# yeeecheng/DA-CLIP

Hardware: AMD Instinct MI355X
Metric: restored images/sec @256x256, 100 IR-SDE steps; PSNR vs ref; 1/2/4/8 MI355X (higher is better)
Workload: dtype fp16; 1 GPU; deraining-shaped synthetic batch, 256x256, batch=8/GPU, 100 IR-SDE posterior steps, hipGraph loop (BASELINE configs[1]); model=universal-ir, batch_per_gpu=8, global_batch=8, resolution=256, sde_steps=100, sampler=posterior, parallelism=dp1

## Files before the change

da-clip_amd/csrc/kernels.h:

```cpp
#pragma once
#include <hip/hip_runtime.h>
#include <stdint.h>

namespace dac {

enum Act { ACT_NONE = 0, ACT_SILU = 1, ACT_GELU = 2, ACT_GEGLU = 3 };

struct ConvArgs {
  const void* x1; const void* x2;
  int ld1, ld2, C1, Cin;
  int Hs, Ws, up;
  int B, Ho, Wo, Cout, K;
  const void* w;
  const float* bias;
  const float* ss;
  int ss_ld;
  const void* res1; int ldr1;
  const void* res2; int ldr2;
  const float* bbias; int bb_ld;
  void* y; int ldy;
  int act;
  int amode;
  long long w_bstride;
  const void* zero;
  const float* ln_g;
  float ln_eps;
  int cwrap;
  const void* w2;
  const float* bias2;
  int w2_dual;
  void* y2; int ldy2;
  const float* lnf_cs;
  int lnf_n;
  float lnf_eps;
  const float* gna_stats;
  const float* gna_g;
  const float* gna_b;
  int gna_groups;
  int dbuf;
  int gna_nb;
  float gna_eps;
  uint8_t* ys8;
  const uint8_t* xs8;
  int uph;
  int ksplit;
  float* part;
  const void* w_gs;
  const float* b_gs;
  unsigned long long* stamp;
};
bool conv_lnf_ok(const ConvArgs& a, int elem_bytes);
bool conv_gna_ok(const ConvArgs& a, int elem_bytes);
template <typename T>
const float* groupnorm_stats(const void* x, int B, int HW, int C, int groups, float eps, float* part,
                             hipStream_t st);
template <typename T>
int layernorm_gnstats(const void* x, int ldx, void* y, int ldy, const float* g, const float* b, int rows, int C,
                      float eps, int HW, int groups, float* part, bool launch, hipStream_t st);
size_t layernorm_gnstats_ws_floats(int B, int HW, int groups);
bool conv_res_fusable(const ConvArgs& a);

inline bool conv3w_ok(const ConvArgs& a) {
  return a.Cin == 64 && a.Cout == 64 && a.K == 576 && a.cwrap == 0 && !a.y2 && (!a.ss || (a.ss_ld % 4 == 0 && ((uintptr_t)a.ss & 15) == 0)) && a.amode == 0 && a.w_bstride == 0 &&
         !a.ln_g && (a.act == ACT_NONE || a.act == ACT_SILU) && a.Wo >= 64 && a.Wo % 64 == 0 &&
         (a.C1 >= a.Cin || a.C1 % 32 == 0) && a.ldy % 8 == 0 && a.ld1 % 8 == 0 &&
         (a.C1 >= a.Cin || a.ld2 % 8 == 0) && (!a.res1 || a.ldr1 % 8 == 0) && !a.res2 && !a.bbias && !(a.ss && a.res1);
}
template <typename T>
void conv(const ConvArgs& a, int kh, int kw, int stride, int pad, hipStream_t st);
struct RbArgs {
  const void* x1; const void* x2;
  int ld1, ld2, C1, Cin;
  int B, H, W;
  const void* w1;
  const void* w2;
  const void* wr;
  const float* ss; int ss_ld;
  void* y; int ldy;
  unsigned long long* stamp;
};
bool rbfuse_pays(const RbArgs& a);
bool rbfuse_ok(const RbArgs& a);
template <typename T>
void rbfuse(const RbArgs& a, hipStream_t st);
bool conv3r_ok(const ConvArgs& a);
template <typename T>
void conv3r(const ConvArgs& a, hipStream_t st);
bool conv7_ok(const ConvArgs& a);
template <typename T>
void conv7(const ConvArgs& a, hipStream_t st);
bool conv3n_ok(const ConvArgs& a);
template <typename T>
void conv3n(const ConvArgs& a, hipStream_t st);
bool conv_down_ok(const ConvArgs& a);
template <typename T>
void conv_down(const ConvArgs& a, hipStream_t st);
int conv_variant(const ConvArgs& a, int kh, int elem_bytes);

bool conv8_ok(const ConvArgs& a, int kh, int kw, int s, int p);
template <typename T>
void conv8(const ConvArgs& a, int kh, int kw, int s, int p, const uint8_t* w8, const uint8_t* ws8, int Kp,
           hipStream_t st);
bool conv_q8out_ok(const ConvArgs& a);
int conv_split_k(const ConvArgs& a, int elem_bytes, long rows);
bool conv3_split_ok(const ConvArgs& a, int elem_bytes);
int conv3_split_k(const ConvArgs& a, int elem_bytes, int ks);
template <typename T>
void conv_part_reduce(const ConvArgs& a, hipStream_t st);
bool conv_uph_ok(const ConvArgs& a, int elem_bytes);
bool conv3q_ok(const ConvArgs& a);
template <typename T>
void conv3q(const ConvArgs& a, const uint8_t* q8w, const uint8_t* q8s, hipStream_t st);

template <typename T>
void layernorm(const void* x, int ldx, void* y, int ldy, const void* res, int ldr,
               const float* g, const float* b, int rows, int C, float eps, hipStream_t st);

template <typename T>
void groupnorm(const void* x, void* y, const float* g, const float* b, int B, int HW, int C,
               int groups, float eps, float* stats_ws, hipStream_t st);

template <typename T>
void flash_attn_d32(const void* qkv, void* o, int B, int L, int H, float scale, hipStream_t st);
template <typename T>
void flash_attn_d32_v(const void* qkv, void* o, int B, int L, int H, float scale, int variant, hipStream_t st);
extern int g_flash_old;

template <typename T>
void text_embed(const int64_t* tok, const float* emb, const float* pos, void* x, int N, int L, int D, int V,
                hipStream_t st);
template <typename T>
void eot_gather(const int64_t* tok, const void* x, void* out, int N, int L, int D, hipStream_t st);
void degradation_probs(const float* degra, const float* text, int B, int K, int E, float* probs,
                       int32_t* argmax, hipStream_t st);

template <typename T>
void small_mha(const void* qkv, void* o, int B, int L, int H, int D, int causal, hipStream_t st);

template <typename T>
void linear_attention_weff(const void* qkv, const float* wout, void* weff, int B, int HW, int C,
                           float* ws, hipStream_t st, float hw_scale = 0.f);
template <typename T>
void linear_attention_fused(const void* x, const void* wqkv, const float* wout, const float* bout,
                            const float* gout, void* weff, void* y, int B, int HW, int C, float* ws,
                            hipStream_t st, float qshift = 0.f);
size_t linear_attention_fused_ws_floats(int B, int HW);
size_t linear_attention_ws_floats(int B, int HW);

void small_linear(const float* x, int ldx, const float* W, const float* b, float* y, int ldy,
                  int R, int I, int O, int pre_act, int post_act, const float* add, int add_ld,
                  int add_mod, hipStream_t st);
void sinus_embedding(float* out, int R, int B, int nf, double t0, double dt, double scale,
                     hipStream_t st);
void round_bf16_rows(float* y, int ld, size_t rows, int C, hipStream_t st);
void ss_fill(float* ss, int C, float scale_m1, const float* shift, hipStream_t st);
void set_u64x2(uint64_t* p, uint64_t a, uint64_t b, hipStream_t st);
void stamp_init(unsigned long long* s, size_t n, hipStream_t st);
void softmax_mul(const float* x, const float* v, float* y, int R, int C, hipStream_t st);

template <typename T>
void unet_prep(const float* xt, const float* mu, void* x, int B, int H, int W, int Hp, int Wp,
               hipStream_t st);

template <typename T>
void unet_out(const void* y, int ld, float* eps, int B, int H, int W, int Hp, int Wp,
              hipStream_t st);

struct StepCoef { float sbar, ea, t1, t2, std, theta, sigma2, dt, sigma_sqrt_dt; };
template <typename T>
void sde_step(int mode, float* x, const float* mu, const void* eps, int ld, int Hp, int Wp,
              const float* z, const uint64_t* seedp, uint32_t tag, StepCoef c, int B, int H,
              int W, hipStream_t st, void* xin = nullptr);
bool sde_step_fuses(int ld, int H, int W, int Hp, int Wp);

void tile_gather(const float* src, float* dst, const int32_t* ys_dev, const int32_t* xs_dev,
                 const int32_t* xs_host, int ny, int nx, int H, int W, int th, int tw, int k0, int nk,
                 hipStream_t st);
void tile_blend(const float* tiles, float* out, const int32_t* ys_dev, const int32_t* xs_dev,
                const int32_t* xs_host, int B, int ny, int nx, int H, int W, int th, int tw, int ov,
                hipStream_t st);
void rows_gather(const float* src, float* dst, int rows, int ld, int k0, int per, hipStream_t st);

template <typename T>
void vit_prep(const float* img, void* x, int B, int S, hipStream_t st);
template <typename T>
void vit_patches(const float* img, void* x, int B, int S, int P, hipStream_t st);
template <typename T>
void vit_embed(const void* patch, const float* cls, const float* pos, void* tok, int B, int L,
               int D, hipStream_t st);
template <typename T>
void rows_to_f32(const void* x, int ld, float* y, int R, int D, hipStream_t st);

bool image_metrics_ok(int B, int C, int H, int W, int cb);
size_t image_metrics_ws_bytes(int B, int C, int H, int W, int cb);
void image_metrics(const float* out, const float* gt, int B, int C, int H, int W, int cb,
                   unsigned char* out_u8, unsigned char* gt_u8, double* results, void* ws,
                   hipStream_t st);

}
```

da-clip_amd/csrc/rbfuse.hip:

```cpp
#include "conv_impl.h"

namespace dac {

namespace {
constexpr unsigned RBF_OOB = 0x80000000u;
DEV int rbf_phys(int p) { return p ^ ((p >> 2) & 1); }
DEV int rbf_chunk(int P, int q) { return q ^ ((P >> 2) & 7); }
DEV int rbf_off(int p, int q) {
  const int P = rbf_phys(p);
  return P * 128 + (rbf_chunk(P, q) << 4);
}

template <int CIN> struct RBF {
  static constexpr int NSRC = CIN / 64;
  static constexpr int SW = CIN == 64 ? 128 : 64;
  static constexpr int NG = SW / 64;
  static constexpr int JT = NG;
  static constexpr int OPW = 16 * JT;
  static constexpr int NGW = 4 / NG;
  static constexpr int NC1 = CIN / 32;
  static constexpr int XPX = SW + 4, NIX = (XPX + 7) / 8, XHALF = NIX * 1024, XROW = NSRC * XHALF;
  static constexpr int HPX = SW + 2, NIH = (HPX + 7) / 8, HROW = NIH * 1024;
  static constexpr int XS = 5, HS = 4;
  static constexpr int OFF_H = XS * XROW, OFF_T = OFF_H + HS * HROW;
  static constexpr int SMEM = OFF_T + 512;
  static_assert(SMEM <= 160 * 1024, "LDS");
};

template <typename T> DEV void store4_g(T* p, const float* v) {
  typedef T T4 __attribute__((ext_vector_type(4)));
  T4 o;
#pragma unroll
  for (int e = 0; e < 4; ++e) o[e] = (T)v[e];
  *reinterpret_cast<T4*>(p) = o;
}
template <typename T> DEV void st_lds(char* p, const float* v, int n) {
  if (n == 8) {
    typedef T T8 __attribute__((ext_vector_type(8)));
    T8 o;
#pragma unroll
    for (int e = 0; e < 8; ++e) o[e] = (T)v[e];
    *reinterpret_cast<T8*>(p) = o;
  } else {
    typedef T T4 __attribute__((ext_vector_type(4)));
    T4 o;
#pragma unroll
    for (int e = 0; e < 4; ++e) o[e] = (T)v[e];
    *reinterpret_cast<T4*>(p) = o;
  }
}
}

static int g_rbfuse_on = getenv("DAC_RBFUSE") ? atoi(getenv("DAC_RBFUSE")) : 1;
extern "C" void dac_rbfuse_enable(int on) { g_rbfuse_on = on; }

bool rbfuse_pays(const RbArgs& a) {
  const size_t px = (size_t)a.B * a.H * a.W, img = (size_t)256 * 256;
  if (g_rbfuse_on == 3) return a.Cin == 64 || px <= 2 * img;
  return true;
}

bool rbfuse_ok(const RbArgs& a) {
  if (!g_rbfuse_on || !(a.Cin == 64 || a.Cin == 128)) return false;
  const int SW = a.Cin == 64 ? RBF<64>::SW : RBF<128>::SW;
  if ((a.Cin == 128) != (a.wr != nullptr)) return false;
  const bool one = a.x2 == nullptr || a.C1 >= a.Cin;
  if (!one && !(a.C1 == 64 && a.Cin == 128 && a.ld2 % 8 == 0)) return false;
  return a.W % SW == 0 && a.W >= 256 && a.ld1 % 8 == 0 && a.ldy % 8 == 0 && a.ss_ld % 4 == 0 &&
         ((size_t)a.H * a.W + 1) * a.ld1 * 2 < ((size_t)1 << 31) &&
         (one || ((size_t)a.H * a.W + 1) * a.ld2 * 2 < ((size_t)1 << 31));
}

template <typename T, int CIN>
__global__ void __launch_bounds__(512, 2) rbfuse_kernel(RbArgs a, int RB) {
  kernarg_touch<sizeof(RbArgs) + 4>();
  StampGuard stamp_guard(a.stamp);
  using G = RBF<CIN>;
  constexpr int JT = G::JT, SW = G::SW, NC1 = G::NC1, EV = 4 * JT;
  constexpr bool FUSE = CIN == 128;
  __shared__ __attribute__((aligned(1024))) char smem[G::SMEM];
  const int lane = threadIdx.x & 63;
  const int wave = __builtin_amdgcn_readfirstlane(threadIdx.x >> 6);
  const bool conv1 = wave < 4;
  const int wl = wave & 3;
  const int g = wl / G::NGW, ob = G::OPW * (wl % G::NGW);
  const int lr = lane & 15, lg = lane >> 4;
  const int nb = ob + EV * lg;

  const int nbands = gridDim.x;
  const int bid = nbands % 8 == 0 ? (blockIdx.x & 7) * (nbands >> 3) + (blockIdx.x >> 3) : blockIdx.x;
  const int S = a.W / SW, nrb = a.H / RB;
  const int strip = bid % S, rb = (bid / S) % nrb, img = bid / (S * nrb);
  const int x0 = strip * SW, r0 = rb * RB;
  const bool lpad = x0 == 0, rpad = x0 + SW == a.W;

  char* xring = smem;
  char* hring = smem + G::OFF_H;
  float* terms = reinterpret_cast<float*>(smem + G::OFF_T);
  if (threadIdx.x < 64) {
    const int n = threadIdx.x;
    float sc = 1.f + a.ss[(size_t)img * a.ss_ld + n], sh = a.ss[(size_t)img * a.ss_ld + 64 + n];
    epi_fold(0.f, sc, sh, true);
    terms[n] = sc;
    terms[64 + n] = sh;
  }

  const bool one = a.x2 == nullptr || a.C1 >= a.Cin;
  const int ldb0 = a.ld1 * 2, ldb1 = one ? ldb0 : a.ld2 * 2;
  const char* xsrc0 = reinterpret_cast<const char*>(a.x1) + (size_t)img * a.H * a.W * ldb0 - 2 * ldb0;
  const char* xsrc1 = one ? xsrc0 + 128
                          : reinterpret_cast<const char*>(a.x2) + (size_t)img * a.H * a.W * ldb1 - 2 * ldb1;
  const int xb0 = (a.H * a.W + 2) * ldb0, xb1 = (a.H * a.W + 2) * ldb1 - (one ? 128 : 0);
  auto xslot = [&](int row) { return xring + ((row + 10) % G::XS) * G::XROW; };
  auto issue_x = [&](int ir) {
    const bool ok = (unsigned)ir < (unsigned)a.H;
    char* dst = xslot(ir);
    int lane = threadIdx.x & 63;
    asm volatile("" : "+v"(lane));
    constexpr int NQ = G::NSRC * G::NIX;
#pragma unroll
    for (int k = 0; k < (NQ + 3) / 4; ++k) {
      const int q = wl + 4 * k;
      if (q < NQ) {
        const bool h1 = q >= G::NIX;
        const int qq = h1 ? q - G::NIX : q, ldb = h1 ? ldb1 : ldb0;
        const int P = 8 * qq + (lane >> 3), p = rbf_phys(P);
        const bool pad = p >= SW + 4 || (lpad && p < 2) || (rpad && p >= SW + 2);
        const int v = (ok && !pad) ? p * ldb + rbf_chunk(P, lane & 7) * 16 : (int)RBF_OOB;
        buf_lds16(h1 ? xsrc1 : xsrc0, h1 ? xb1 : xb0, dst + q * 1024, v, ok ? (ir * a.W + x0) * ldb : 0);
      }
    }
  };

  auto quad_base = [&](int u) {
    const int q = lr + u;
    return (64 * g + 4 * q) * 128 + ((q & 1) << 7) + ((lg ^ ((16 * g + q) & 7)) << 4);
  };
  const int bq0 = quad_base(0), bq1 = quad_base(1);
  auto foff = [&](int b0, int b1, int s, int c) {
    const int base = s < 4 ? b0 : b1;
    return base ^ ((s & 3) << 7) ^ (c << 6);
  };

  const int nsteps = RB + 3;
  if (conv1) {
    u32x4 W[9 * NC1][JT];
    {
      const T* w = reinterpret_cast<const T*>(a.w1);
#pragma unroll
      for (int j = 0; j < JT; ++j) {
        const int n = JT == 2 ? ob + 8 * (lr >> 2) + 4 * j + (lr & 3) : ob + lr;
#pragma unroll
        for (int ks = 0; ks < 9 * NC1; ++ks)
          W[ks][j] = *reinterpret_cast<const u32x4*>(w + (size_t)n * (9 * CIN) + (ks / NC1) * CIN + (ks % NC1) * 32 + 8 * lg);
      }
    }
    __builtin_amdgcn_s_waitcnt(0x0F70);
    issue_x(r0 - 2);
    issue_x(r0 - 1);
    issue_x(r0);
    int eoff[3], fo[2][6];
#pragma unroll
    for (int kw = 0; kw < 3; ++kw) eoff[kw] = rbf_off(lr < 8 ? SW + 1 + kw : kw, lg);
#pragma unroll
    for (int c = 0; c < 2; ++c)
#pragma unroll
      for (int s = 0; s < 6; ++s) fo[c][s] = foff(bq0, bq1, s + 1, c);
    for (int st = 0; st < nsteps; ++st) {
      const int t = r0 - 1 + st;
      asm volatile("s_waitcnt vmcnt(0) lgkmcnt(0)" ::: "memory");
      __builtin_amdgcn_s_barrier();
      asm volatile("" ::: "memory");
      if (t + 2 <= r0 + RB + 1) issue_x(t + 2);
      if (t > r0 + RB) continue;
      char* hdst = hring + (t & 3) * G::HROW;
      if ((unsigned)t >= (unsigned)a.H) {
        for (int i = threadIdx.x; i < G::HROW / 16; i += 256) reinterpret_cast<u32x4*>(hdst)[i] = u32x4{0u, 0u, 0u, 0u};
        continue;
      }
      f32x4 acc[4][JT], acce = f32x4{0.f, 0.f, 0.f, 0.f};
#pragma unroll
      for (int j = 0; j < JT; ++j)
#pragma unroll
        for (int i = 0; i < 4; ++i) acc[i][j] = f32x4{0.f, 0.f, 0.f, 0.f};
      if constexpr (CIN == 128) {
        constexpr int NGR = 3 * NC1;
        u32x4 F2[2][6];
        auto gsrc = [&](int gg) { return xslot(t + gg / NC1 - 1) + ((gg % NC1) >> 1) * G::XHALF; };
        auto ldF = [&](int gg, int h) __attribute__((always_inline)) {
          const char* hr = gsrc(gg);
          const int c = (gg % NC1) & 1;
#pragma unroll
          for (int s = 0; s < 6; ++s) F2[h][s] = *reinterpret_cast<const u32x4*>(hr + fo[c][s]);
        };
        ldF(0, 0);
#pragma unroll
        for (int gg = 0; gg < NGR; ++gg) {
          const int kh = gg / NC1, c32 = gg % NC1, c = c32 & 1;
          const char* hr = gsrc(gg);
          if (gg + 1 < NGR) ldF(gg + 1, (gg + 1) & 1);
          __builtin_amdgcn_sched_barrier(0);
#pragma unroll
          for (int kw = 0; kw < 3; ++kw)
#pragma unroll
            for (int i = 0; i < 4; ++i) Mma<T>::run(acc[i][0], W[(kh * 3 + kw) * NC1 + c32][0], F2[gg & 1][i + kw]);
#pragma unroll
          for (int kw = 0; kw < 3; ++kw) {
            const u32x4 E = *reinterpret_cast<const u32x4*>(hr + (eoff[kw] ^ (c << 6)));
            Mma<T>::run(acce, W[(kh * 3 + kw) * NC1 + c32][0], E);
          }
        }
      } else {
        constexpr int NGR = 3 * NC1;
        auto gsrc = [&](int gg) { return xslot(t + gg / NC1 - 1) + ((gg % NC1) >> 1) * G::XHALF; };
        u32x4 F[6];
        {
          const char* hr0 = gsrc(0);
#pragma unroll
          for (int s = 0; s < 6; ++s) F[s] = *reinterpret_cast<const u32x4*>(hr0 + fo[0][s]);
        }
        constexpr int H1[6][2] = {{0, 0}, {0, 1}, {1, 0}, {0, 2}, {1, 1}, {2, 0}};
        constexpr int H2[6][2] = {{1, 2}, {2, 1}, {3, 0}, {2, 2}, {3, 1}, {3, 2}};
#pragma unroll
        for (int gg = 0; gg < NGR; ++gg) {
          const int kh = gg / NC1, c32 = gg % NC1, c = c32 & 1;
          const char* hr = gsrc(gg);
          const char* hn = gsrc(gg + 1 < NGR ? gg + 1 : gg);
          const int cn = ((gg + 1) % NC1) & 1;
          __builtin_amdgcn_sched_barrier(0);
#pragma unroll
          for (int q = 0; q < 6; ++q)
#pragma unroll
            for (int j = 0; j < JT; ++j)
              Mma<T>::run(acc[H1[q][0]][j], W[(kh * 3 + H1[q][1]) * NC1 + c32][j], F[H1[q][0] + H1[q][1]]);
          __builtin_amdgcn_sched_barrier(0);
          if (gg + 1 < NGR) {
#pragma unroll
            for (int s = 0; s < 3; ++s) F[s] = *reinterpret_cast<const u32x4*>(hn + fo[cn][s]);
          }
          __builtin_amdgcn_sched_barrier(0);
#pragma unroll
          for (int q = 0; q < 6; ++q)
#pragma unroll
            for (int j = 0; j < JT; ++j)
              Mma<T>::run(acc[H2[q][0]][j], W[(kh * 3 + H2[q][1]) * NC1 + c32][j], F[H2[q][0] + H2[q][1]]);
          __builtin_amdgcn_sched_barrier(0);
          if (gg + 1 < NGR) {
#pragma unroll
            for (int s = 3; s < 6; ++s) F[s] = *reinterpret_cast<const u32x4*>(hn + fo[cn][s]);
          }
#pragma unroll
          for (int kw = 0; kw < 3; ++kw) {
            const u32x4 E = *reinterpret_cast<const u32x4*>(hr + (eoff[kw] ^ (c << 6)));
            if (JT == 1 || g == 0) Mma<T>::run(acce, W[(kh * 3 + kw) * NC1 + c32][0], E);
            else Mma<T>::run(acce, W[(kh * 3 + kw) * NC1 + c32][JT - 1], E);
          }
        }
      }
      __builtin_amdgcn_sched_barrier(0);
      float fs[EV], fh[EV];
      {
        const f32x4* tv = reinterpret_cast<const f32x4*>(terms + nb);
#pragma unroll
        for (int q = 0; q < JT; ++q) {
          const f32x4 s0 = tv[q], h0 = tv[16 + q];
#pragma unroll
          for (int e = 0; e < 4; ++e) { fs[4 * q + e] = s0[e]; fh[4 * q + e] = h0[e]; }
        }
      }
      const int q16 = nb >> 3, half8 = (nb >> 2) & 1;
#pragma unroll
      for (int i = 0; i < 4; ++i) {
        float v[EV];
#pragma unroll
        for (int e = 0; e < EV; ++e) v[e] = silu_log2(fmaf(acc[i][e >> 2][e & 3], fs[e], fh[e]));
        st_lds<T>(hdst + rbf_off(64 * g + 4 * lr + i + 1, q16) + half8 * 8, v, EV);
      }
      {
        const bool zero = lr < 8 ? rpad : lpad;
        const int jg = JT == 1 ? 0 : g;
        float v[4];
#pragma unroll
        for (int e = 0; e < 4; ++e) {
          const float sc = jg ? fs[EV - 4 + e] : fs[e], sh = jg ? fh[EV - 4 + e] : fh[e];
          v[e] = zero ? 0.f : silu_log2(fmaf(acce[e], sc, sh));
          asm volatile("" : "+v"(v[e]));
        }
        st_lds<T>(hdst + rbf_off(lr < 8 ? SW + 1 : 0, q16) + (half8 + jg) * 8, v, 4);
      }
    }
  } else {
    u32x4 W[18][JT];
    u32x4 WR[FUSE ? NC1 : 1][JT];
    {
      const T* w = reinterpret_cast<const T*>(a.w2);
#pragma unroll
      for (int j = 0; j < JT; ++j) {
        const int n = JT == 2 ? ob + 8 * (lr >> 2) + 4 * j + (lr & 3) : ob + lr;
#pragma unroll
        for (int ks = 0; ks < 18; ++ks)
          W[ks][j] = *reinterpret_cast<const u32x4*>(w + (size_t)n * 576 + (ks >> 1) * 64 + (ks & 1) * 32 + 8 * lg);
        if constexpr (FUSE) {
          const T* wr = reinterpret_cast<const T*>(a.wr);
#pragma unroll
          for (int c = 0; c < NC1; ++c) WR[c][j] = *reinterpret_cast<const u32x4*>(wr + (size_t)n * CIN + c * 32 + 8 * lg);
        }
      }
    }
    __builtin_amdgcn_s_waitcnt(0x0F70);
    T* y = reinterpret_cast<T*>(a.y);
    const int q16 = nb >> 3;
    int fo[2][6];
#pragma unroll
    for (int c = 0; c < 2; ++c)
#pragma unroll
      for (int s = 0; s < 6; ++s) fo[c][s] = foff(bq0, bq1, s, c);
    for (int st = 0; st < nsteps; ++st) {
      const int t = r0 - 1 + st, u = t - 2;
      asm volatile("s_waitcnt lgkmcnt(0)" ::: "memory");
      __builtin_amdgcn_s_barrier();
      asm volatile("" ::: "memory");
      if (u < r0) continue;
      f32x4 acc[4][JT];
#pragma unroll
      for (int i = 0; i < 4; ++i)
#pragma unroll
        for (int j = 0; j < JT; ++j) acc[i][j] = f32x4{0.f, 0.f, 0.f, 0.f};
      {
        auto hsrc = [&](int gg) { return hring + ((u + gg / 2 - 1) & 3) * G::HROW; };
        constexpr int H1[6][2] = {{0, 0}, {0, 1}, {1, 0}, {0, 2}, {1, 1}, {2, 0}};
        constexpr int H2[6][2] = {{1, 2}, {2, 1}, {3, 0}, {2, 2}, {3, 1}, {3, 2}};
        u32x4 F[6];
        {
          const char* h0 = hsrc(0);
#pragma unroll
          for (int s = 0; s < 6; ++s) F[s] = *reinterpret_cast<const u32x4*>(h0 + fo[0][s]);
        }
#pragma unroll
        for (int gg = 0; gg < 6; ++gg) {
          const int kh = gg / 2, c = gg & 1, cn = (gg + 1) & 1;
          const char* hn = hsrc(gg + 1 < 6 ? gg + 1 : gg);
          __builtin_amdgcn_sched_barrier(0);
#pragma unroll
          for (int q = 0; q < 6; ++q)
#pragma unroll
            for (int j = 0; j < JT; ++j)
              Mma<T>::run(acc[H1[q][0]][j], W[(kh * 3 + H1[q][1]) * 2 + c][j], F[H1[q][0] + H1[q][1]]);
          __builtin_amdgcn_sched_barrier(0);
          if (gg + 1 < 6) {
#pragma unroll
            for (int s = 0; s < 3; ++s) F[s] = *reinterpret_cast<const u32x4*>(hn + fo[cn][s]);
          }
          __builtin_amdgcn_sched_barrier(0);
#pragma unroll
          for (int q = 0; q < 6; ++q)
#pragma unroll
            for (int j = 0; j < JT; ++j)
              Mma<T>::run(acc[H2[q][0]][j], W[(kh * 3 + H2[q][1]) * 2 + c][j], F[H2[q][0] + H2[q][1]]);
          __builtin_amdgcn_sched_barrier(0);
          if (gg + 1 < 6) {
#pragma unroll
            for (int s = 3; s < 6; ++s) F[s] = *reinterpret_cast<const u32x4*>(hn + fo[cn][s]);
          }
        }
      }
      f32x4 accr[FUSE ? 4 : 1][JT];
      if constexpr (FUSE) {
#pragma unroll
        for (int i = 0; i < 4; ++i)
#pragma unroll
          for (int j = 0; j < JT; ++j) accr[i][j] = f32x4{0.f, 0.f, 0.f, 0.f};
        const char* xr = xslot(u);
#pragma unroll
        for (int c32 = 0; c32 < NC1; ++c32) {
          __builtin_amdgcn_sched_barrier(0);
          const char* hr = xr + (c32 >> 1) * G::XHALF;
          u32x4 F[4];
#pragma unroll
          for (int i = 0; i < 4; ++i) F[i] = *reinterpret_cast<const u32x4*>(hr + fo[c32 & 1][i + 2]);
#pragma unroll
          for (int i = 0; i < 4; ++i)
#pragma unroll
            for (int j = 0; j < JT; ++j) Mma<T>::run(accr[i][j], WR[c32][j], F[i]);
        }
      }
      __builtin_amdgcn_sched_barrier(0);
      const size_t m0 = ((size_t)img * a.H + u) * a.W + x0 + 64 * g + 4 * lr;
#pragma unroll
      for (int i = 0; i < 4; ++i) {
        float v[EV];
#pragma unroll
        for (int e = 0; e < EV; ++e) v[e] = silu_log2(acc[i][e >> 2][e & 3] * kL2E);
        if constexpr (FUSE) {
#pragma unroll
          for (int w2 = 0; w2 < EV / 2; ++w2) {
            const T lo = from_f<T>(accr[i][(2 * w2) >> 2][(2 * w2) & 3]);
            const T hi = from_f<T>(accr[i][(2 * w2 + 1) >> 2][(2 * w2 + 1) & 3]);
            const unsigned u = (unsigned)__builtin_bit_cast(unsigned short, lo) |
                               ((unsigned)__builtin_bit_cast(unsigned short, hi) << 16);
            add_pair<T>(u, v[2 * w2], v[2 * w2 + 1]);
          }
          store4_g<T>(y + (m0 + i) * a.ldy + nb, v);
        } else {
          const u32x4 r = *reinterpret_cast<const u32x4*>(xslot(u) + rbf_off(64 * g + 4 * lr + i + 2, q16));
#pragma unroll
          for (int w2 = 0; w2 < 4; ++w2) add_pair<T>(r[w2], v[2 * w2], v[2 * w2 + 1]);
          store_vec<T>(y + (m0 + i) * a.ldy + nb, v);
        }
      }
    }
  }
  asm volatile("s_waitcnt vmcnt(0)" ::: "memory");
}

static int rbfuse_rb(const RbArgs& a, int SW) {
  const long rows = (long)a.B * a.H * (a.W / SW);
  int rb = (int)(rows / 256);
  if (rb < 1) rb = 1;
  if (rb > a.H) rb = a.H;
  while (a.H % rb) --rb;
  return rb;
}

template <typename T>
void rbfuse(const RbArgs& a, hipStream_t st) {
  if (!rbfuse_ok(a)) throw std::invalid_argument("rbfuse: arguments rejected by rbfuse_ok");
  if (a.Cin == 64) {
    const int rb = rbfuse_rb(a, RBF<64>::SW);
    rbfuse_kernel<T, 64><<<a.B * (a.H / rb) * (a.W / RBF<64>::SW), 512, 0, st>>>(a, rb);
  } else {
    const int rb = rbfuse_rb(a, RBF<128>::SW);
    rbfuse_kernel<T, 128><<<a.B * (a.H / rb) * (a.W / RBF<128>::SW), 512, 0, st>>>(a, rb);
  }
}
template void rbfuse<bf16>(const RbArgs&, hipStream_t);
template void rbfuse<f16>(const RbArgs&, hipStream_t);

}
```

Measured before the change: 28.35 images/s.

## Batch rbfuse CIN=128 edge-column conv over NB rows via dedicated LDS ring

For the 128-channel fused resblock kernel, the per-row edge (halo column) convolution is replaced with a batched scheme. A separate LDS ring prefetches edge input rows ahead. Every NB rows the edge outputs for NB rows are computed at once, with each lane owning one row, and kept in registers until written. This removes the per-row edge MMA work and its LDS reads from the main loop, at the cost of more LDS, extra async loads and extra registers, which may lower occupancy.

Result: no change. 28.19 images/s (-0.6%).

```diff
diff --git a/da-clip_amd/csrc/kernels.h b/da-clip_amd/csrc/kernels.h
--- a/da-clip_amd/csrc/kernels.h
+++ b/da-clip_amd/csrc/kernels.h
@@ -81,6 +81,7 @@
 };
 bool rbfuse_pays(const RbArgs& a);
 bool rbfuse_ok(const RbArgs& a);
+int rbfuse_band_rows(const RbArgs& a);
 template <typename T>
 void rbfuse(const RbArgs& a, hipStream_t st);
 bool conv3r_ok(const ConvArgs& a);
diff --git a/da-clip_amd/csrc/rbfuse.hip b/da-clip_amd/csrc/rbfuse.hip
--- a/da-clip_amd/csrc/rbfuse.hip
+++ b/da-clip_amd/csrc/rbfuse.hip
@@ -23,8 +23,11 @@
   static constexpr int HPX = SW + 2, NIH = (HPX + 7) / 8, HROW = NIH * 1024;
   static constexpr int XS = 5, HS = 4;
   static constexpr int OFF_H = XS * XROW, OFF_T = OFF_H + HS * HROW;
-  static constexpr int SMEM = OFF_T + 512;
+  static constexpr int NB = CIN == 128 ? 8 : 0;
+  static constexpr int ES = 2 * NB, EROW = 2048, OFF_E = OFF_T + 512;
+  static constexpr int SMEM = OFF_E + (NB ? ES * EROW : 0);
   static_assert(SMEM <= 160 * 1024, "LDS");
+  static_assert(NB == 0 || ((NB == 4 || NB == 8) && ES >= NB + 3 && (ES & (ES - 1)) == 0), "edge ring");
 };
 
 template <typename T> DEV void store4_g(T* p, const float* v) {
@@ -131,6 +134,21 @@
       }
     }
   };
+  char* ering = smem + G::OFF_E;
+  auto issue_e = [&](int ir) {
+    const bool ok = (unsigned)ir < (unsigned)a.H;
+    int lane = threadIdx.x & 63;
+    asm volatile("" : "+v"(lane));
+    const bool h1 = wl & 1;
+    const int ldb = h1 ? ldb1 : ldb0;
+    const int kw = lane >> 4, side = (lane >> 1) & 1;
+    const int q = ((((lane >> 2) & 3) ^ (ir & 3)) << 1) | (lane & 1);
+    const int p = side ? SW + 1 + kw : kw;
+    const bool pad = kw > 2 || (lpad && p < 2) || (rpad && p >= SW + 2);
+    const int v = (ok && !pad) ? p * ldb + q * 16 : (int)RBF_OOB;
+    buf_lds16(h1 ? xsrc1 : xsrc0, h1 ? xb1 : xb0, ering + (ir & (G::ES - 1)) * G::EROW + h1 * 1024, v,
+              ok ? (ir * a.W + x0) * ldb : 0);
+  };
 
   auto quad_base = [&](int u) {
     const int q = lr + u;
@@ -159,6 +177,15 @@
     issue_x(r0 - 2);
     issue_x(r0 - 1);
     issue_x(r0);
+    constexpr int NB = G::NB, NBD = NB ? NB : 1;
+    typedef uint32_t u32x2 __attribute__((ext_vector_type(2)));
+    const int elast = r0 - 1 + (RB + 1) / NBD * NBD + NB;
+    const int eside = (lr / NBD) & 1;
+    u32x2 ekeep = u32x2{0u, 0u};
+    if constexpr (NB != 0) {
+#pragma unroll
+      for (int j = 0; j < (NB + 2) / 2; ++j) issue_e(r0 - 2 + 2 * j + (wl >> 1));
+    }
     int eoff[3], fo[2][6];
 #pragma unroll
     for (int kw = 0; kw < 3; ++kw) eoff[kw] = rbf_off(lr < 8 ? SW + 1 + kw : kw, lg);
@@ -172,8 +199,50 @@
       __builtin_amdgcn_s_barrier();
       asm volatile("" ::: "memory");
       if (t + 2 <= r0 + RB + 1) issue_x(t + 2);
+      if constexpr (NB != 0) {
+        if (wl >= 2 && t + NB + 1 <= elast) issue_e(t + NB + 1);
+      }
       if (t > r0 + RB) continue;
       char* hdst = hring + (t & 3) * G::HROW;
+      if constexpr (NB != 0) {
+        if ((st & (NB - 1)) == 0) {
+          int eo[3][2];
+#pragma unroll
+          for (int kh = 0; kh < 3; ++kh) {
+            const int rw = t + (lr & (NB - 1)) + kh - 1;
+            eo[kh][0] = ((rw & (G::ES - 1)) * G::EROW) | (((rw & 3) ^ (lg >> 1)) << 6) | (eside << 5) | ((lg & 1) << 4);
+            eo[kh][1] = eo[kh][0] ^ 128;
+          }
+          constexpr int NGR = 3 * NC1;
+          u32x4 E2[2][3];
+          auto ldE = [&](int gg, int h) __attribute__((always_inline)) {
+            const char* er = ering + ((gg % NC1) >> 1) * 1024 + eo[gg / NC1][(gg % NC1) & 1];
+#pragma unroll
+            for (int kw = 0; kw < 3; ++kw) E2[h][kw] = *reinterpret_cast<const u32x4*>(er + kw * 256);
+          };
+          f32x4 accb = f32x4{0.f, 0.f, 0.f, 0.f};
+          ldE(0, 0);
+#pragma unroll
+          for (int gg = 0; gg < NGR; ++gg) {
+            const int kh = gg / NC1, c32 = gg % NC1;
+            if (gg + 1 < NGR) ldE(gg + 1, (gg + 1) & 1);
+#pragma unroll
+            for (int kw = 0; kw < 3; ++kw) Mma<T>::run(accb, W[(kh * 3 + kw) * NC1 + c32][0], E2[gg & 1][kw]);
+          }
+          const f32x4 es = *reinterpret_cast<const f32x4*>(terms + nb), eh = *reinterpret_cast<const f32x4*>(terms + 64 + nb);
+          const bool zero = eside ? rpad : lpad;
+          typedef T T4 __attribute__((ext_vector_type(4)));
+          T4 o;
+#pragma unroll
+          for (int e = 0; e < 4; ++e) {
+            float v = zero ? 0.f : silu_log2(fmaf(accb[e], es[e], eh[e]));
+            asm volatile("" : "+v"(v));
+            o[e] = (T)v;
+          }
+          ekeep = __builtin_bit_cast(u32x2, o);
+          __builtin_amdgcn_sched_barrier(0);
+        }
+      }
       if ((unsigned)t >= (unsigned)a.H) {
         for (int i = threadIdx.x; i < G::HROW / 16; i += 256) reinterpret_cast<u32x4*>(hdst)[i] = u32x4{0u, 0u, 0u, 0u};
         continue;
@@ -196,19 +265,13 @@
         ldF(0, 0);
 #pragma unroll
         for (int gg = 0; gg < NGR; ++gg) {
-          const int kh = gg / NC1, c32 = gg % NC1, c = c32 & 1;
-          const char* hr = gsrc(gg);
+          const int kh = gg / NC1, c32 = gg % NC1;
           if (gg + 1 < NGR) ldF(gg + 1, (gg + 1) & 1);
           __builtin_amdgcn_sched_barrier(0);
 #pragma unroll
           for (int kw = 0; kw < 3; ++kw)
 #pragma unroll
             for (int i = 0; i < 4; ++i) Mma<T>::run(acc[i][0], W[(kh * 3 + kw) * NC1 + c32][0], F2[gg & 1][i + kw]);
-#pragma unroll
-          for (int kw = 0; kw < 3; ++kw) {
-            const u32x4 E = *reinterpret_cast<const u32x4*>(hr + (eoff[kw] ^ (c << 6)));
-            Mma<T>::run(acce, W[(kh * 3 + kw) * NC1 + c32][0], E);
-          }
         }
       } else {
         constexpr int NGR = 3 * NC1;
@@ -276,7 +339,10 @@
         for (int e = 0; e < EV; ++e) v[e] = silu_log2(fmaf(acc[i][e >> 2][e & 3], fs[e], fh[e]));
         st_lds<T>(hdst + rbf_off(64 * g + 4 * lr + i + 1, q16) + half8 * 8, v, EV);
       }
-      {
+      if constexpr (NB != 0) {
+        if (lr < 2 * NB && (lr & (NB - 1)) == (st & (NB - 1)))
+          *reinterpret_cast<u32x2*>(hdst + rbf_off(eside ? SW + 1 : 0, q16) + half8 * 8) = ekeep;
+      } else {
         const bool zero = lr < 8 ? rpad : lpad;
         const int jg = JT == 1 ? 0 : g;
         float v[4];
@@ -421,6 +487,7 @@
   while (a.H % rb) --rb;
   return rb;
 }
+int rbfuse_band_rows(const RbArgs& a) { return rbfuse_rb(a, a.Cin == 64 ? RBF<64>::SW : RBF<128>::SW); }
 
 template <typename T>
 void rbfuse(const RbArgs& a, hipStream_t st) {
```
